# sevagh/demucs.cpp

Hardware: AMD Instinct MI355X
Metric: audio-sec/s (xRT) htdemucs-4s 44.1kHz stereo, ~4-min track with overlap-add (BASELINE configs[2]) (higher is better)
Workload: dtype f32 (exact bf16x3 operand split, fp32 accumulate)

## Files before the change

demucs_cpp_amd/csrc/api.cpp:

```cpp
#include "api_internal.h"

#include <algorithm>
#include <atomic>
#include <cstdarg>
#include <cstdio>
#include <cstdlib>
#include <cmath>
#include <cstring>
#include <cctype>
#include <cerrno>
#include <climits>
#include <fcntl.h>
#include <pthread.h>
#include <signal.h>
#include <sys/mman.h>
#include <sys/stat.h>
#include <unistd.h>

using namespace dmx;

static thread_local std::string g_err;
int dmx_fail(int code, const char *fmt, ...)
{
    char buf[1024];
// ... 108 lines not shown
    float *dx = nullptr;
    unsigned short *dp = nullptr;
    HIPCHK(hipMalloc((void **)&dx, sizeof(float) * (size_t)n));
    hipError_t e = hipMalloc((void **)&dp, sizeof(unsigned short) * 3 * (size_t)n);
    if (e == hipSuccess)
        e = hipMemcpy(dx, x, sizeof(float) * (size_t)n, hipMemcpyHostToDevice);
    if (e == hipSuccess)
    {
        launch_split3h_debug(dx, n, scale_exp, dp, nullptr);
        e = hipMemcpy(planes, dp, sizeof(unsigned short) * 3 * (size_t)n, hipMemcpyDeviceToHost);
    }
    (void)hipFree(dx);
    if (dp)
        (void)hipFree(dp);
    if (e != hipSuccess)
        return fail(DMX_ERR_HIP, "dmx_debug_split_activations_fp16: %s", hipGetErrorString(e));
    return DMX_OK;
}

static void fill_gemm_geometry(GemmArgs &k, const IGemm &g)
{
    k.xBS = g.xBatchStride;
    k.B = g.B, k.P1 = g.P1, k.P0 = g.P0, k.L1 = g.L1, k.L0 = g.L0, k.Cin = g.Cin;
    k.S1 = g.S1, k.stride1 = g.stride1, k.dil1 = g.dil1, k.pad1 = g.pad1;
    k.seg0 = g.seg0, k.stride0 = g.stride0, k.pad0 = g.pad0, k.K = g.K, k.Kp = g.Kp;
    k.pro = g.pro, k.G0 = g.G0;
    k.N = g.N, k.Np = g.Np;
    k.epi = g.epi, k.act = g.act, k.yBS = g.yBatchStride, k.ldy = g.ldy;
    k.NB = g.NB, k.tableScale = g.tableScale;
    k.Lout = g.Lout, k.Cout = g.Cout, k.trS = g.trS, k.trOff = g.trOff;
    k.kvCol0 = g.kvCol0, k.kvT = g.kvT, k.kvH = g.kvH, k.kvHs = g.kvHs;
    k.M = (i64)g.B * g.P1 * g.P0;
}

static bool split_ok_model(const dmx_ctx *c, const dmx_model *m, const IGemm &g);
static bool split_ok(const dmx_ctx *c, const IGemm &g) { return split_ok_model(c, c->m, g); }
static bool split_ok_model(const dmx_ctx *c, const dmx_model *m, const IGemm &g)
{
    if (c->gemm == DMX_GEMM_F32 || !m->dWb)
        return false;
    GemmArgs k{};
    fill_gemm_geometry(k, g);
    k.Wb1 = m->dWb + g.w_w, k.Wb2 = m->dWb + m->blobFloats + 512 + g.w_w;
    if (launch_igemm_split(g.cfg, k, nullptr, true) != 0)
        return false;
    const i64 lo = g.w_w, hi = g.w_w + (i64)g.Np * g.Kp;
    auto it = std::lower_bound(m->inexactW.begin(), m->inexactW.end(), lo);
    return it == m->inexactW.end() || *it >= hi;
}

static int split_kind_model(const dmx_ctx *c, const dmx_model *m, const IGemm &g)
{
    if (!split_ok_model(c, m, g))
        return 0;
    if (c->gemm != DMX_GEMM_FP16X3 || !m->dWh || !g.hterms)
        return 1;
    GemmArgs k{};
    fill_gemm_geometry(k, g);
    k.Wb1 = k.Wb2 = m->dWh;
    if (launch_igemm_split(g.cfg, k, nullptr, true, 1) != 0)
        return 1;
    const i64 lo = g.w_w, hi = g.w_w + (i64)g.Np * g.Kp;
    auto it = std::lower_bound(m->inexactH.begin(), m->inexactH.end(), lo);
    return (it == m->inexactH.end() || *it >= hi) ? 2 : 1;
}
static int split_kind(const dmx_ctx *c, const IGemm &g) { return split_kind_model(c, c->m, g); }

static int upload_failed(dmx_model *m, hipError_t e)
{
    for (void *p : {(void *)m->dW, (void *)m->dWb, (void *)m->dWh})
        if (p)
            (void)hipFree(p);
    m->dW = nullptr, m->dWb = nullptr, m->dWh = nullptr;
    return fail(DMX_ERR_HIP, "dmx_model_load: weight upload failed: %s", hipGetErrorString(e));
}

int dmx_model_upload(dmx_model *m, const float *blob)
{
    HIPCHK(hipSetDevice(m->device));
    HIPCHK(hipMalloc((void **)&m->dW, m->blobFloats * sizeof(float) + 1024));
    hipError_t e = hipMemset(reinterpret_cast<char *>(m->dW) + m->blobFloats * sizeof(float), 0, 1024);
    if (e == hipSuccess)
        e = hipMemcpy(m->dW, blob, m->blobFloats * sizeof(float), hipMemcpyHostToDevice);
    if (e != hipSuccess)
        return upload_failed(m, e);
    {
        std::vector<unsigned short> planes(2 * m->blobFloats + 1024, 0);
        m->inexactW.clear();
        for (size_t i = 0; i < m->blobFloats; ++i)
            if (!dmx_split_weight(blob[i], planes[i], planes[m->blobFloats + 512 + i]))
                m->inexactW.push_back((i64)i);
// ... 1602 lines not shown
extern "C" int dmx_debug_n_ops(const dmx_ctx *c)
{
    if (!c)
        return 0;
    auto it = c->plans.find(c->maxBatch);
    return it == c->plans.end() ? 0 : (int)it->second->ops.size();
}

static void op_work(const Op &op, const char *&kernel, double &flops, double &bytes)
{
    static const char *cfgNames[] = {"igemm_128x128", "igemm_64x64", "igemm_128x96", "igemm_128x48", "igemm_256x16", "igemm_128x32",
                                     "igemm_128x64",  "igemm_64x128", "dgemm_direct", "igemm_64x64", "igemm_64x96", "igemm_64x48",
                                     "igemm_64x32",   "igemm_64x64",  "igemm_128x16", "igemm_32x128", "igemm_32x64", "igemm_256x128", "igemm_256x128w4", "igemm_lin256x128", "igemm_256x96"};
    static_assert(sizeof(cfgNames) / sizeof(cfgNames[0]) == kNumTileCfgs, "one label per tile configuration");
    flops = bytes = 0;
    kernel = "?";
    switch (op.kind)
    {
    case OP_IGEMM:
    {
        const IGemm &g = op.g;
        const double M = (double)g.B * g.P1 * g.P0;
        kernel = cfgNames[g.cfg];
        if (g.split)
        {
            static const char *splitNames[kNumTileCfgs] = {"igemm_split_128x128", nullptr, "igemm_split_128x96", "igemm_split_128x48", nullptr, "igemm_split_128x32d", "igemm_split_128x64d",
                                                            "igemm_split_64x128", nullptr, "igemm_split_64x64", "igemm_split_64x96", "igemm_split_64x48",
                                                            "igemm_split_128x32d", "igemm_split_128x64d", nullptr, "igemm_split_32x128", "igemm_split_32x64", nullptr, nullptr,
                                                            nullptr, nullptr};
            if (splitNames[g.cfg])
                kernel = splitNames[g.cfg];
            if (g.split == 2)
                kernel = g.cfg == 0 ? "igemm_splith_128x128" : g.cfg == 7 ? "igemm_splith_64x128" : kernel;
            else if (g.cfg == 0 || g.cfg == 2)
            {
                GemmArgs k{};
                fill_gemm_geometry(k, g);
                k.rowstat = g.rowstat >= 0 ? reinterpret_cast<float *>(1) : nullptr;
                const int wide = igemm_split_is_wide(g.cfg, k);
                if (wide)
                    kernel = wide == 256 ? "igemm_split_128x256" : wide == 192 ? "igemm_split_128x192" : "igemm_split_128x96d";
            }
        }
        flops = 2.0 * M * g.N * g.K;
        double in = (double)g.B * g.L1 * g.L0 * g.Cin, w = (double)g.N * g.K, out = 0;
        if (g.epi == EPI_LINEAR || g.epi == EPI_SCALE_RES)
            out = M * g.N;
        else if (g.epi == EPI_KPL || g.epi == EPI_VT)
            out = M * g.N;
        else if (g.epi == EPI_GLU || g.epi == EPI_GN_GLU_SCALE_RES)
            out = M * g.N / 2;
        else if (g.epi == EPI_TRCONV)
            out = (double)g.B * g.P1 * g.Lout * g.Cout;
        double res = g.res >= 0 ? out : 0;
        bytes = 4.0 * (in + w + out + res);
        break;
    }
    case OP_ATTENTION:
    {
        const Attention &t = op.at;
        kernel = t.split ? "attention_split" : "attention";
        flops = 4.0 * t.B * t.H * (double)t.Tq * t.Tk * t.hs;
        bytes = 4.0 * t.B * t.H * t.hs * (2.0 * t.Tq + 2.0 * t.Tk);
        break;
    }
    case OP_DCONV_ROW:
    {
        const DconvRow &r = op.dr;
        const double M = (double)r.B * r.T * r.F, hp = (r.hid + 3) / 4 * 4;
        kernel = "dconv_row";
        flops = 2.0 * (2.0 * M * hp * 3.0 * r.C + 2.0 * M * (hp + 2) * hp + 2.0 * M * 2.0 * r.C * hp);
        bytes = 4.0 * 2.0 * M * r.C;
        break;
    }
// ... 120 lines not shown
```

demucs_cpp_amd/csrc/igemm_common.h:

```cpp
#pragma once
#include "kernels.h"

namespace dmx
{

typedef float f32x4 __attribute__((ext_vector_type(4)));
typedef float f32x2 __attribute__((ext_vector_type(2)));
typedef unsigned u32x4 __attribute__((ext_vector_type(4)));
typedef unsigned u32x2 __attribute__((ext_vector_type(2)));
typedef __bf16 bf16x2 __attribute__((ext_vector_type(2)));
typedef __bf16 bf16x8 __attribute__((ext_vector_type(8)));

__device__ __forceinline__ float gelu_f(float v) { return dmx_gelu(v); }
__device__ __forceinline__ float sigmoid_f(float v) { return __builtin_amdgcn_rcpf(1.0f + __expf(-v)); }
__device__ __forceinline__ float f4c(const f32x4 &v, int c) { return v[c]; }
__device__ __forceinline__ float4 ld4z(const float *ptr, bool ok, const float *zero)
{
    const f32x4 v = *reinterpret_cast<const f32x4 *>(ok ? ptr : zero);
    return make_float4(v[0], v[1], v[2], v[3]);
}

__device__ __forceinline__ void load_to_lds_b128(const float *gptr, float4 *lds_base)
{
#if defined(__HIP_DEVICE_COMPILE__)
// ... 272 lines not shown
                addrs_B();
            return;
        }
        if (c < 2)
            addrs_A_general(c);
        if (c == 2)
            addrs_B();
    }
    __device__ __forceinline__ f32x4 transform(f32x4 v, int i, bool ok, const f32x4 &gW, const f32x4 &gB) const
    {
        if (PRO != PRO_NONE)
        {
            if (PRO == PRO_AFFINE)
            {
                v.x = (v.x - aMean[i]) * aScale[i];
                v.y = (v.y - aMean[i]) * aScale[i];
                v.z = (v.z - aMean[i]) * aScale[i];
                v.w = (v.w - aMean[i]) * aScale[i];
            }
            if (PRO == PRO_GN_GELU)
            {
                v.x = gelu_f((v.x - aMean[i]) * aScale[i] * gW.x + gB.x);
                v.y = gelu_f((v.y - aMean[i]) * aScale[i] * gW.y + gB.y);
                v.z = gelu_f((v.z - aMean[i]) * aScale[i] * gW.z + gB.z);
                v.w = gelu_f((v.w - aMean[i]) * aScale[i] * gW.w + gB.w);
            }
            if (!ok)
                v = f32x4{0.f, 0.f, 0.f, 0.f};
        }
        return v;
    }
};

template <int WAVES_N, int WMF, int WNF, int EPI, int NT, int SSEG = 1, typename RowInfo>
__device__ __forceinline__ void igemm_epilogue(const GemmArgs &p, f32x4 (&acc)[WMF][WNF], RowInfo rowinfo, float2 (*rsum)[WAVES_N * SSEG], i64 m0,
                                               int n0, unsigned tileN, int wm, int wn, int BM)
{
    static_assert(WNF % SSEG == 0, "whole fragments per statistics run");
    const int tid = threadIdx.x, lane = tid & 63;
    const int l15 = lane & 15, kq = lane >> 4;
    if constexpr (EPI == EPI_VT)
    {
        const int nt = p.kvT >> 6;
        constexpr int IS = (WMF % 2 == 0) ? 2 : 1;
#pragma unroll
        for (int i = 0; i < WMF; i += IS)
        {
            const i64 m = m0 + wm * (WMF * 16) + i * 16 + 4 * kq;
            if (m >= p.M)
                continue;
            const unsigned b = (unsigned)m / (unsigned)p.kvT, t = (unsigned)m - b * (unsigned)p.kvT;
            const unsigned tt = t & 63u, slot = 4u * (tt >> 5) + ((tt >> 2) & 3u), half = (tt >> 4) & 1u;
#pragma unroll
            for (int j = 0; j < WNF; ++j)
            {
                const int n = n0 + wn * (WNF * 16) + j * 16 + l15;
                if (n >= p.N)
                    continue;
                const float bv = p.bias[n];
                const unsigned head = (unsigned)n / (unsigned)p.kvHs, dim = (unsigned)n - head * (unsigned)p.kvHs;
                unsigned short *dst = p.kvPl + ((((i64)b * p.kvH + head) * nt + (t >> 6)) * p.kvHs + dim) * 64 + slot * 8;
                unsigned h1[2 * IS], h2[2 * IS], h3[2 * IS];
#pragma unroll
                for (int u = 0; u < IS; ++u)
                {
                    split3_pk(acc[i + u][j][0] + bv, acc[i + u][j][1] + bv, h1[2 * u], h2[2 * u], h3[2 * u]);
                    split3_pk(acc[i + u][j][2] + bv, acc[i + u][j][3] + bv, h1[2 * u + 1], h2[2 * u + 1], h3[2 * u + 1]);
                }
                if constexpr (IS == 2)
// ... 41 lines not shown
                            *reinterpret_cast<float4 *>(p.Y + m * p.ldy + nb + 16 * u + 4 * kq) = v[u];
                    continue;
                }
                unsigned h[3][2][2];
#pragma unroll
                for (int u = 0; u < 2; ++u)
                {
                    split3_pk(v[u].x, v[u].y, h[0][u][0], h[1][u][0], h[2][u][0]);
                    split3_pk(v[u].z, v[u].w, h[0][u][1], h[1][u][1], h[2][u][1]);
                }
                const int nn = nb + 16 * (kq & 1) + 8 * (kq >> 1);
                unsigned short *dst = p.kvPl + m * (i64)(p.kvH * p.kvHs) + (nn - p.kvCol0);
#pragma unroll
                for (int pl = 0; pl < 3; ++pl)
                {
                    const u32x2 s0 = __builtin_amdgcn_permlane16_swap(h[pl][0][0], h[pl][1][0], false, false);
                    const u32x2 s1 = __builtin_amdgcn_permlane16_swap(h[pl][0][1], h[pl][1][1], false, false);
                    if (rowOk && nn < p.N)
                        *reinterpret_cast<u32x4 *>(dst + pl * p.kvPlane) = u32x4{s0[0], s1[0], s0[1], s1[1]};
                }
            }
        }
        return;
    }
    const bool wantStats = p.rowstat != nullptr;
    const int colBase = n0 + wn * (WNF * 16) + 4 * kq;
    float4 biasv[WNF], scalev[WNF], gnWv[WNF], gnBv[WNF];
    int trR[WNF], trC[WNF];
#pragma unroll
    for (int j = 0; j < WNF; ++j)
    {
        const int n = colBase + j * 16;
        const float4 z = make_float4(0.f, 0.f, 0.f, 0.f);
        biasv[j] = ld4z(p.bias + n, n < p.N, p.zero);
        scalev[j] = gnWv[j] = gnBv[j] = z;
        trR[j] = trC[j] = 0;
        if (EPI == EPI_TRCONV)
        {
            trR[j] = n / p.Cout;
            trC[j] = n - trR[j] * p.Cout;
        }
        if (EPI == EPI_SCALE_RES && n < p.N)
            scalev[j] = *reinterpret_cast<const float4 *>(p.scale + n);
        if (EPI == EPI_GN_GLU_SCALE_RES && n < p.N)
        {
            gnWv[j] = *reinterpret_cast<const float4 *>(p.epiW + n);
            gnBv[j] = *reinterpret_cast<const float4 *>(p.epiB + n);
            if ((j & 1) == 0)
                scalev[j] = *reinterpret_cast<const float4 *>(p.scale + (n >> 5) * 16 + (n & 15));
        }
    }

    constexpr int G = (16 / WNF) < 1 ? 1 : ((16 / WNF) > WMF ? WMF : (16 / WNF));
    int4 riA[G];
    float4 resA[G][WNF];
    float meanA[G], scA[G];
    i64 offsA[G][WNF];
#pragma unroll
    for (int g0 = 0; g0 < WMF; g0 += G)
    {
#pragma unroll
    for (int ig = 0; ig < G; ++ig)
    {
        const int i = g0 + ig;
        if (i >= WMF)
            break;
        const int rl = wm * (WMF * 16) + i * 16 + l15;
// ... 6 lines not shown
        for (int j = 0; j < WNF; ++j)
            resA[ig][j] = make_float4(0.f, 0.f, 0.f, 0.f);
        if (EPI == EPI_LINEAR || EPI == EPI_SCALE_RES)
        {
            if ((EPI == EPI_LINEAR && p.res) || EPI == EPI_SCALE_RES)
            {
#pragma unroll
                for (int j = 0; j < WNF; ++j)
                {
                    const int n = colBase + j * 16;
                    if (rowOk && n < p.N)
                        resA[ig][j] = *reinterpret_cast<const float4 *>(p.res + m * p.ldy + n);
                }
            }
        }
        else if (EPI == EPI_GLU || EPI == EPI_GN_GLU_SCALE_RES)
        {
            if (EPI == EPI_GN_GLU_SCALE_RES && rowOk)
            {
                meanA[ig] = p.epiStats[ri.w * 4];
                scA[ig] = p.epiStats[ri.w * 4 + 1];
            }
#pragma unroll
            for (int j = 0; j < WNF; j += 2)
            {
                const int na = colBase + j * 16;
                const int c = (na >> 5) * 16 + (na & 15);
                if (rowOk && na + 16 < p.N)
                {
                    if (EPI == EPI_GN_GLU_SCALE_RES)
                        resA[ig][j] = *reinterpret_cast<const float4 *>(p.res + m * p.ldy + c);
                    else if (p.table)
                    {
                        const float4 tv = *reinterpret_cast<const float4 *>(p.table + (i64)ri.z * (p.N >> 1) + c);
                        resA[ig][j] = make_float4(p.tableScale * tv.x, p.tableScale * tv.y, p.tableScale * tv.z, p.tableScale * tv.w);
                    }
                }
            }
        }
        else if (EPI == EPI_TRCONV)
        {
#pragma unroll
            for (int j = 0; j < WNF; ++j)
            {
                const int n = colBase + j * 16;
                const int jj = p.trS * ri.z + trR[j] - p.trOff;
                const i64 off = (rowOk && n < p.N && jj >= 0 && jj < p.Lout) ? (i64)ri.x * p.yBS + ((i64)ri.y * p.Lout + jj) * p.ldy + trC[j] : -1;
                offsA[ig][j] = off;
                if (p.res && off >= 0)
                    resA[ig][j] = *reinterpret_cast<const float4 *>(p.res + off);
            }
        }
    }
    __builtin_amdgcn_s_waitcnt(0x0F70);

#pragma unroll
    for (int ig = 0; ig < G; ++ig)
    {
        const int i = g0 + ig;
        if (i >= WMF)
            break;
        const int rl = wm * (WMF * 16) + i * 16 + l15;
        const int4 ri = riA[ig];
        const bool rowOk = ri.w >= 0;
        const i64 m = m0 + rl;
        float s = 0.f, ss = 0.f;
        float sSeg[SSEG], ssSeg[SSEG];
// ... 161 lines not shown
```

demucs_cpp_amd/csrc/igemm_split.hip:

```cpp
#include "igemm_common.h"
#include <cstdio>
#include <cstdlib>
#include <type_traits>

namespace dmx
{

__device__ __forceinline__ int swz(int row) { return (0x1320 >> (((row >> 2) & 3) * 4)) & 3; }

template <int WAVES_M, int WAVES_N, int WMF, int WNF, int PRO, int EPI, bool LIN>
__global__ __launch_bounds__(256, 2) void igemm_split_kernel(const GemmArgs p)
{
    constexpr int KT = 32;
    constexpr int BM = WAVES_M * WMF * 16;
    constexpr int BN = WAVES_N * WNF * 16;
    constexpr int LPR = 8;
    constexpr int RP = 256 / LPR;
    constexpr int AR = BM / RP;
    constexpr int BR = (BN + RP - 1) / RP;
    constexpr int BRP = BR * RP;
    static_assert(WAVES_M * WAVES_N == 4, "256 threads");
    static_assert(BM % RP == 0, "BM multiple of the staging pass");

    __shared__ u32x4 Ap0[3][BM][4], Ap1[3][BM][4];
// ... 386 lines not shown
            iteration(set1);
    }
    __syncthreads();
    if constexpr (ARITH == 1)
    {
#pragma unroll
        for (int i = 0; i < WMF; ++i)
        {
            if constexpr (EPI == EPI_VT)
            {
                float inv[4];
#pragma unroll
                for (int r = 0; r < 4; ++r)
                    inv[r] = p.rowScale[2 * min(m0 + wave * (WMF * 16) + i * 16 + 4 * kq + r, p.M - 1) + 1];
#pragma unroll
                for (int j = 0; j < WNF; ++j)
#pragma unroll
                    for (int r = 0; r < 4; ++r)
                        acc[i][j][r] *= inv[r];
            }
            else
            {
#pragma unroll
                for (int j = 0; j < WNF; ++j)
#pragma unroll
                    for (int r = 0; r < 4; ++r)
                        acc[i][j][r] *= aInv[i];
            }
        }
    }
    igemm_epilogue<1, WMF, WNF, EPI, 256, 2>(p, acc, rowinfo_of, rsum, m0, n0, tileN, wave, 0, BM);
}

template <int WNF, int EPI, bool GEN>
__global__ __launch_bounds__(256, WNF == 2 ? 4 : WNF <= 6 ? 3 : 2) void igemm_split_linw_kernel(const GemmArgs p)
{
    constexpr int KT = 32, WMF = 2, BM = 128, BN = 16 * WNF, NG = WNF / 2;
    constexpr int PW = WNF / 2;
    static_assert(WNF == 16 || WNF == 12 || WNF == 6 || WNF == 4 || WNF == 2,
                  "128 x 256 / 128 x 192 / 128 x 96 (N = 96 layers: three workgroups per CU) / 128 x 64 (the last transposed conv of the "
                  "frequency branch, N = 64: three) / 128 x 32 (the C = 192 DConv K1, N = 24: four)");
    __shared__ u32x4 Bp[2][2][BN][4];

    const int tid = threadIdx.x, lane = tid & 63, wave = tid >> 6;
    const int l15 = lane & 15, kq = lane >> 4;
    unsigned tileM, tileN;
    if (!tile_of_block(p, tileM, tileN))
        return;
    const i64 m0 = (i64)tileM * BM;
    const int n0 = (int)tileN * BN;
    auto rowinfo_of = [&](int r) -> int4 { return row_info(p, m0 + r); };

    unsigned aOff[WMF];
    const float *aRow[WMF];
    unsigned aMask[WMF];
    int gS1 = 0, gOffb = kq * 8, gTapC = 0, gTapOff = kq * 8;
    const int rowLenI = p.L0 * p.Cin;
    {
        const i64 rowLen = (i64)p.L0 * p.Cin;
#pragma unroll
        for (int i = 0; i < WMF; ++i)
        {
            const i64 m = min(m0 + wave * (WMF * 16) + i * 16 + l15, p.M - 1);
            const int4 ri = row_info(p, m);
            aOff[i] = 0, aRow[i] = p.X, aMask[i] = 0;
            if constexpr (GEN)
            {
                const int taps0 = p.seg0 / p.Cin;
                const int in1_0 = ri.y * p.stride1 - p.pad1;
                const int e0 = (ri.z * p.stride0 - p.pad0) * p.Cin;
                aRow[i] = p.X + (i64)ri.x * p.xBS + (i64)in1_0 * rowLen + e0;
                unsigned m0bits = 0;
                for (int t0 = 0; t0 < taps0; ++t0)
                {
                    const int e = e0 + t0 * p.Cin;
                    m0bits |= (e >= 0 && e < rowLenI ? 1u : 0u) << t0;
                }
                for (int s = 0; s < p.S1; ++s)
                {
                    const int in1 = in1_0 + s * p.dil1;
                    if (in1 >= 0 && in1 < p.L1)
                        aMask[i] |= m0bits << (s * taps0);
                }
            }
            else
                aOff[i] = (unsigned)(((i64)ri.x * p.xBS + (i64)ri.y * rowLen + (i64)ri.z * p.stride0 * p.Cin) * 4 + kq * 32);
        }
        if constexpr (GEN)
        {
            if (p.S1 > 1)
                while (gOffb >= p.seg0)
                {
                    gOffb -= p.seg0;
                    ++gS1;
                }
            while (gTapOff >= p.Cin)
            {
                gTapOff -= p.Cin;
// ... 56 lines not shown
            aRaw[SET][i][0] = *reinterpret_cast<const f32x4 *>(src);
            aRaw[SET][i][1] = *reinterpret_cast<const f32x4 *>(src + 16);
            aOff[i] += KT * 4;
        }
    };
    auto split_block = [&](auto setTag, int i) {
        constexpr int SET = decltype(setTag)::value;
        const f32x4 lo = aRaw[SET][i][0], hi = aRaw[SET][i][1];
        unsigned h1[4], h2[4], h3[4];
        split3_pk(lo[0], lo[1], h1[0], h2[0], h3[0]);
        split3_pk(lo[2], lo[3], h1[1], h2[1], h3[1]);
        split3_pk(hi[0], hi[1], h1[2], h2[2], h3[2]);
        split3_pk(hi[2], hi[3], h1[3], h2[3], h3[3]);
        u32x4 q1{h1[0], h1[1], h1[2], h1[3]}, q2{h2[0], h2[1], h2[2], h2[3]}, q3{h3[0], h3[1], h3[2], h3[3]};
        asm volatile("" : "+v"(q1), "+v"(q2), "+v"(q3));
        aPl[SET][i][0] = q1;
        aPl[SET][i][1] = q2;
        aPl[SET][i][2] = q3;
    };

    f32x4 acc[WMF][WNF];
#pragma unroll
    for (int i = 0; i < WMF; ++i)
#pragma unroll
        for (int j = 0; j < WNF; ++j)
            acc[i][j] = f32x4{0.f, 0.f, 0.f, 0.f};

    const std::integral_constant<int, 0> set0{};
    const std::integral_constant<int, 1> set1{};
    const int nk = (p.Kp + 31) >> 5;
    load_A(set0);
    load_A(set1);
    dma_B(0);
    split_block(set0, 0);
    split_block(set0, 1);
    asm volatile("s_waitcnt vmcnt(0)" ::: "memory");
    __syncthreads();
    const int fslot = kq ^ swz(l15);
    auto iteration = [&](auto parTag) {
        constexpr int PAR = decltype(parTag)::value;
        const std::integral_constant<int, PAR ^ 1> other{};
        load_A(parTag);
        __builtin_amdgcn_sched_barrier(0);
        dma_B(PAR ^ 1);
        u32x4 b1[2][2], b2[2][2];
        auto read_group = [&](int g) {
#pragma unroll
            for (int u = 0; u < 2; ++u)
            {
                const int r = (2 * g + u) * 16 + l15;
                b1[g & 1][u] = Bp[PAR][0][r][fslot];
                b2[g & 1][u] = Bp[PAR][1][r][fslot];
            }
        };
        auto term = [&](int g, u32x4(&b)[2], int plane) {
#pragma unroll
            for (int i = 0; i < WMF; ++i)
#pragma unroll
                for (int u = 0; u < 2; ++u)
                {
                    if constexpr (EPI == EPI_VT)
                        acc[i][2 * g + u] = __builtin_amdgcn_mfma_f32_16x16x32_bf16(__builtin_bit_cast(bf16x8, aPl[PAR][i][plane]), __builtin_bit_cast(bf16x8, b[u]), acc[i][2 * g + u], 0, 0, 0);
                    else
                        acc[i][2 * g + u] = __builtin_amdgcn_mfma_f32_16x16x32_bf16(__builtin_bit_cast(bf16x8, b[u]), __builtin_bit_cast(bf16x8, aPl[PAR][i][plane]), acc[i][2 * g + u], 0, 0, 0);
                }
        };
        read_group(0);
#pragma unroll
        for (int g = 0; g < NG; ++g)
        {
            if (g + 1 < NG)
                read_group(g + 1);
            term(g, b1[g & 1], 2);
            term(g, b2[g & 1], 1);
            if (g == (WNF == 16 ? 2 : WNF == 12 ? 1 : 0))
                split_block(other, 0);
            if (g == (WNF == 16 ? 5 : WNF == 12 ? 4 : WNF == 6 ? 2 : WNF == 4 ? 1 : 0))
                split_block(other, 1);
            term(g, b2[g & 1], 0);
            term(g, b1[g & 1], 1);
            term(g, b1[g & 1], 0);
            __builtin_amdgcn_sched_barrier(0);
        }
        asm volatile("s_waitcnt vmcnt(0)" ::: "memory");
        __syncthreads();
    };
    for (int kt = 0; kt < nk; kt += 2)
    {
        iteration(set0);
        if (kt + 1 < nk)
            iteration(set1);
    }

    if constexpr (EPI == EPI_KPL || EPI == EPI_VT)
    {
        float2(*none)[1] = nullptr;
        igemm_epilogue<1, WMF, WNF, EPI, 256>(p, acc, rowinfo_of, none, m0, n0, tileN, wave, 0, BM);
    }
    else if constexpr (WNF == 2)
    {
        float2(*rsum)[1] = reinterpret_cast<float2(*)[1]>(&Bp[0][0][0][0]);
        igemm_epilogue<1, WMF, WNF, EPI, 256>(p, acc, rowinfo_of, rsum, m0, n0, tileN, wave, 0, BM);
    }
    else if constexpr (GEN || WNF != 16)
    {
        float2(*none)[1] = nullptr;
        constexpr int JC = WNF % 4 == 0 ? 4 : 6;
#pragma unroll
        for (int jc = 0; jc < WNF; jc += JC)
        {
            f32x4 part[WMF][JC];
#pragma unroll
            for (int i = 0; i < WMF; ++i)
#pragma unroll
                for (int j = 0; j < JC; ++j)
                    part[i][j] = acc[i][jc + j];
            igemm_epilogue<1, WMF, JC, EPI, 256>(p, part, rowinfo_of, none, m0, n0 + 16 * jc, tileN, wave, 0, BM);
        }
    }
    else
    {
        static_assert(EPI == EPI_LINEAR || EPI == EPI_SCALE_RES, "plain linear layers");
        const bool hasRes = EPI == EPI_SCALE_RES || p.res != nullptr;
        const bool wantStats = p.rowstat != nullptr;
        float2(*rsum)[4] = reinterpret_cast<float2(*)[4]>(&Bp[0][0][0][0]);
#pragma unroll
        for (int jc = 0; jc < WNF; jc += 4)
        {
            float4 biasv[4], scalev[4], resv[WMF][4];
#pragma unroll
            for (int j = 0; j < 4; ++j)
            {
                const int n = n0 + (jc + j) * 16 + 4 * kq;
                biasv[j] = *reinterpret_cast<const float4 *>(p.bias + n);
                if (EPI == EPI_SCALE_RES)
                    scalev[j] = *reinterpret_cast<const float4 *>(p.scale + n);
#pragma unroll
                for (int i = 0; i < WMF; ++i)
                {
                    const i64 m = m0 + wave * (WMF * 16) + i * 16 + l15;
                    resv[i][j] = make_float4(0.f, 0.f, 0.f, 0.f);
                    if (hasRes && m < p.M)
                        resv[i][j] = *reinterpret_cast<const float4 *>(p.res + m * p.ldy + n);
                }
            }
#pragma unroll
            for (int i = 0; i < WMF; ++i)
            {
                const int rl = wave * (WMF * 16) + i * 16 + l15;
                const i64 m = m0 + rl;
// ... 129 lines not shown
{
    const i64 pairs = (n + 1) / 2;
    hipLaunchKernelGGL(split3h_debug_kernel, dim3((unsigned)((pairs + 255) / 256)), dim3(256), 0, s, d_x, n, ldexpf(1.0f, sexp), d_planes);
}

static constexpr double kWideMinRounds = 2.5;
static bool wide_tile_pays(const GemmArgs &a, int mode)
{
    if (a.N % 256 != 0 || a.Np != a.N || a.Kp % 32 != 0 || mode == 2 || mode == 0 || (a.rowstat && a.NB != a.N / 128))
        return false;
    if (mode == 3)
        return true;
    const i64 tm = (a.M + 127) / 128;
    return (double)(((tm + 7) / 8) * (a.N / 256)) / 64.0 >= kWideMinRounds;
}

static int wide_conv_width(const GemmArgs &a, int pro, int epi, int mode)
{
    if (mode == 0 || mode == 2 || pro != PRO_NONE || !(epi == EPI_LINEAR || epi == EPI_GLU || epi == EPI_TRCONV) || a.rowstat)
        return 0;
    const int wnf = a.N % 256 == 0 ? 16 : a.N % 192 == 0 ? 12 : a.N == 96 ? 6 : 0;
    if (!wnf || a.Np != a.N || a.Kp % 16 != 0 || a.Cin % 8 != 0 || a.seg0 % a.Cin != 0 || a.seg0 < 32 || a.S1 * (a.seg0 / a.Cin) > 32 ||
        (i64)a.S1 * a.dil1 * a.L0 * a.Cin + a.seg0 >= (1ll << 31) || (epi == EPI_TRCONV && a.Cout % 4 != 0))
        return 0;
    if (mode == 3)
        return wnf;
    if (mode == 4 && wnf == 6)
        return 0;
    if (wnf == 6)
        return wnf;
    const i64 tm = (a.M + 127) / 128;
    return (double)(((tm + 7) / 8) * (a.N / (16 * wnf))) / 64.0 >= (a.N == 192 ? 0.6 : 0.9) ? wnf : 0;
}
template <int EPI>
static void launch_wide_conv(GemmArgs a, int wnf, hipStream_t s)
{
    a.tilesM = (unsigned)((a.M + 127) / 128);
    a.tilesN = (unsigned)(a.N / (16 * wnf));
    const dim3 grid(8u * ((a.tilesM + 7u) / 8u) * a.tilesN);
    if (wnf == 16)
        hipLaunchKernelGGL((igemm_split_linw_kernel<16, EPI, true>), grid, dim3(256), 0, s, a);
    else if (wnf == 12)
        hipLaunchKernelGGL((igemm_split_linw_kernel<12, EPI, true>), grid, dim3(256), 0, s, a);
    else
        hipLaunchKernelGGL((igemm_split_linw_kernel<6, EPI, true>), grid, dim3(256), 0, s, a);
}

static int launch_split_narrow(int cfg, const GemmArgs &a0, hipStream_t s, int arith, bool dry)
{
    const GemmArgs &a = a0;
    const int np = (cfg == 5 || cfg == 12) ? 32 : 64;
    if (arith != 0 || a.pro != PRO_NONE || !(a.epi == EPI_LINEAR || (a.epi == EPI_TRCONV && np == 64)) || (a.epi == EPI_LINEAR && a.res) || a.N > np || a.Np != np ||
        a.Kp % 16 != 0 || a.Cin % 8 != 0 || a.Cin <= 0 || a.seg0 % a.Cin != 0 || a.seg0 < 32 || a.S1 * (a.seg0 / a.Cin) > 32 ||
        (i64)a.S1 * a.dil1 * a.L0 * a.Cin + a.seg0 >= (1ll << 31) || a.NB != 1 || (a.epi == EPI_TRCONV && (a.rowstat || a.Cout % 4 != 0)) ||
        (np == 64 && a.rowstat))
        return -1;
    if (dry)
        return 0;
    GemmArgs k = a;
    k.tilesM = (unsigned)((k.M + 127) / 128);
    k.tilesN = 1;
    k.xcdMap = 1;
    k.dP0 = make_fastdiv((unsigned)k.P0), k.dP1 = make_fastdiv((unsigned)k.P1);
    const dim3 grid(8u * ((k.tilesM + 7u) / 8u));
    if (np == 32)
        hipLaunchKernelGGL((igemm_split_linw_kernel<2, EPI_LINEAR, true>), grid, dim3(256), 0, s, k);
    else if (a.epi == EPI_LINEAR)
        hipLaunchKernelGGL((igemm_split_linw_kernel<4, EPI_LINEAR, true>), grid, dim3(256), 0, s, k);
    else
        hipLaunchKernelGGL((igemm_split_linw_kernel<4, EPI_TRCONV, true>), grid, dim3(256), 0, s, k);
    return 0;
}

template <int WM_, int WN_, int MF, int NF, int PRO, int EPI>
static int launch_split_one(const GemmArgs &a0, hipStream_t s, int arith, bool dry)
{
    if (dry && arith == 0 && EPI != EPI_KPL && EPI != EPI_VT)
        return 0;
    constexpr int BM = WM_ * MF * 16, BN = WN_ * NF * 16;
    GemmArgs a = a0;
    a.tilesM = (unsigned)((a.M + BM - 1) / BM);
    a.tilesN = (unsigned)((a.N + BN - 1) / BN);
    a.xcdMap = 1;
    a.dP0 = make_fastdiv((unsigned)a.P0), a.dP1 = make_fastdiv((unsigned)a.P1);
    const unsigned blocks = 8u * ((a.tilesM + 7u) / 8u) * a.tilesN;
    const bool lin = gemm_is_linear(a, PRO, EPI, 32) && ((i64)a.B * a.xBS + 64) * 4 < (1ll << 32) &&
                     ((i64)(a.Wb2 - a.Wb1) + (i64)a.Np * a.Kp + 64) * 2 < (1ll << 32);
    if constexpr (EPI == EPI_KPL || EPI == EPI_VT)
    {
        if constexpr (PRO == PRO_NONE && WM_ == 2 && WN_ == 2 && NF == 4 && MF >= 2)
            if (lin)
            {
                if (dry)
                    return 0;
                static const int mode = [] { const char *e = getenv("DMX_SPLIT_LIN"); return e ? atoi(e) : 1; }();
                if (arith == 1)
                    hipLaunchKernelGGL((igemm_split_lin_kernel<MF / 2, 8, EPI, 1>), dim3(blocks), dim3(256), 0, s, a);
                else if (MF == 4 && wide_tile_pays(a, mode == 0 ? 1 : mode))
                {
                    a.tilesN = (unsigned)(a.N / 256);
                    hipLaunchKernelGGL((igemm_split_linw_kernel<16, EPI, false>), dim3(8u * ((a.tilesM + 7u) / 8u) * a.tilesN), dim3(256), 0, s, a);
// ... 45 lines not shown
                return -1;
            hipLaunchKernelGGL((igemm_split_kernel<WM_, WN_, MF, NF, PRO, EPI, true>), dim3(blocks), dim3(256), 0, s, a);
            return 0;
        }
    }
    if (arith == 1)
        return -1;
    if constexpr (PRO == PRO_NONE && EPI == EPI_TRCONV && ((WM_ == 2 && WN_ == 2 && MF == 4 && NF == 4) || (WM_ == 4 && WN_ == 1 && MF == 2 && NF == 6)))
    {
        static const int mode = [] { const char *e = getenv("DMX_SPLIT_LIN"); return e ? atoi(e) : 1; }();
        if (const int wnf = wide_conv_width(a, PRO, EPI, mode))
        {
            launch_wide_conv<EPI>(a, wnf, s);
            return 0;
        }
    }
    if constexpr (EPI != EPI_KPL && EPI != EPI_VT)
        hipLaunchKernelGGL((igemm_split_kernel<WM_, WN_, MF, NF, PRO, EPI, false>), dim3(blocks), dim3(256), 0, s, a);
    return 0;
}

int igemm_split_is_wide(int cfg, const GemmArgs &a)
{
    static const int mode = [] { const char *e = getenv("DMX_SPLIT_LIN"); return e ? atoi(e) : 1; }();
    if (cfg != 0 && cfg != 2)
        return 0;
    const bool lin = gemm_is_linear(a, a.pro, a.epi, 32) && ((i64)a.B * a.xBS + 64) * 4 < (1ll << 32);
    if (cfg == 0 && lin && (a.epi == EPI_LINEAR || a.epi == EPI_SCALE_RES || a.epi == EPI_KPL || a.epi == EPI_VT) &&
        wide_tile_pays(a, (a.epi == EPI_KPL || a.epi == EPI_VT) && mode == 0 ? 1 : mode))
        return 256;
    if (lin && a.epi == EPI_LINEAR && a.N % 256 == 0)
        return 0;
    return 16 * wide_conv_width(a, a.pro, a.epi, mode);
}

int launch_igemm_split(int cfg, const GemmArgs &a, hipStream_t s, bool dry, int arith)
{
    if (a.M >= (1ll << 31) - 256 || !a.Wb1 || !a.Wb2)
        return -1;
#define DMX_CASE(cfgid, WM_, WN_, MF, NF, PRO, EPI) \
    case (cfgid * 100 + PRO * 10 + EPI):           \
        return launch_split_one<WM_, WN_, MF, NF, PRO, EPI>(a, s, arith, dry);
    if (cfg == 5 || cfg == 12 || cfg == 6 || cfg == 13)
        return launch_split_narrow(cfg, a, s, arith, dry);
    switch (cfg * 100 + a.pro * 10 + a.epi)
    {
        DMX_CASE(0, 2, 2, 4, 4, PRO_NONE, EPI_LINEAR)
        DMX_CASE(0, 2, 2, 4, 4, PRO_NONE, EPI_SCALE_RES)
        DMX_CASE(0, 2, 2, 4, 4, PRO_NONE, EPI_GLU)
        DMX_CASE(0, 2, 2, 4, 4, PRO_NONE, EPI_TRCONV)
        DMX_CASE(7, 2, 2, 2, 4, PRO_NONE, EPI_LINEAR)
        DMX_CASE(7, 2, 2, 2, 4, PRO_NONE, EPI_SCALE_RES)
        DMX_CASE(7, 2, 2, 2, 4, PRO_NONE, EPI_GLU)
        DMX_CASE(7, 2, 2, 2, 4, PRO_NONE, EPI_TRCONV)
        DMX_CASE(0, 2, 2, 4, 4, PRO_NONE, EPI_KPL)
        DMX_CASE(0, 2, 2, 4, 4, PRO_NONE, EPI_VT)
        DMX_CASE(7, 2, 2, 2, 4, PRO_NONE, EPI_KPL)
        DMX_CASE(7, 2, 2, 2, 4, PRO_NONE, EPI_VT)
        DMX_CASE(2, 4, 1, 2, 6, PRO_NONE, EPI_LINEAR)
        DMX_CASE(2, 4, 1, 2, 6, PRO_NONE, EPI_GLU)
        DMX_CASE(2, 4, 1, 2, 6, PRO_NONE, EPI_TRCONV)
        DMX_CASE(15, 2, 2, 1, 4, PRO_NONE, EPI_LINEAR)
        DMX_CASE(15, 2, 2, 1, 4, PRO_NONE, EPI_SCALE_RES)
        DMX_CASE(15, 2, 2, 1, 4, PRO_NONE, EPI_GLU)
        DMX_CASE(15, 2, 2, 1, 4, PRO_NONE, EPI_TRCONV)
        DMX_CASE(9, 2, 2, 2, 2, PRO_NONE, EPI_LINEAR)
// ... 20 lines not shown
```

demucs_cpp_amd/csrc/kernels.h:

```cpp
#pragma once
#include "plan.h"
#include <hip/hip_runtime.h>
#include <cstdlib>

namespace dmx
{

struct FastDiv
{
    unsigned magic, shift;
};
inline FastDiv make_fastdiv(unsigned d)
{
    FastDiv f;
    f.magic = 0;
    f.shift = 0;
    if (d == 0)
        d = 1;
    if ((d & (d - 1)) == 0)
    {
        while ((1u << f.shift) < d)
            ++f.shift;
        return f;
    }
// ... 27 lines not shown
    const float *table;
    float tableScale;
    int Lout, Cout;
    int trS, trOff;
    const float *rowScale;
    unsigned short *kvPl;
    i64 kvPlane;
    int kvCol0, kvT, kvH, kvHs;
    i64 M;
    const float *zero;
    unsigned tilesM, tilesN;
    FastDiv dP0, dP1;
    int xcdMap;
};

int launch_dgemm(const GemmArgs &a, hipStream_t s, bool dry = false);

struct DconvRowArgs
{
    float *x;
    int B, T, F, C, hid;
    const float *img[2];
    float eps;
    const float *zero;
    int rowsPerXcd;
    double n1, invN1, invN1m1, n2, invN2, invN2m1;
};
int launch_dconv_row(const DconvRowArgs &a, hipStream_t s, bool dry = false);

int launch_igemm(int cfg, const GemmArgs &a, hipStream_t s, bool dry = false);
int launch_igemm_lin256(const GemmArgs &a, hipStream_t s, bool dry = false);
int launch_igemm_split(int cfg, const GemmArgs &a, hipStream_t s, bool dry = false, int arith = 0);
int igemm_split_is_wide(int cfg, const GemmArgs &a);
void launch_rowscale(const GemmArgs &a, float *out, hipStream_t s);
void launch_split3h_debug(const float *d_x, i64 n, int sexp, unsigned short *d_planes, hipStream_t s);
void launch_split3_debug(const float *d_x, i64 n, unsigned short *d_planes, hipStream_t s);

struct ReduceArgs
{
    const float *rowstat;
    float *out;
    int B, R, NB, G0;
    double count;
    int mode;
    float eps;
    double *scratch;
    int nchunk;
};
void launch_stats_reduce(const ReduceArgs &a, hipStream_t s);

struct StftArgs
{
    const float *mix;
    float *x, *rowstat, *rowstatT;
    int B, T, seg, pad;
    const float *window, *twiddle;
};
void launch_stft(const StftArgs &a, hipStream_t s);

struct LnArgs
{
    const float *x;
    float *y;
    int rows, D, rowsPerBatch;
    const float *w, *b, *pe;
    float eps;
// ... 205 lines not shown
```

Before: 3173.

## Add resident-weight short-K variants of the split wide conv GEMM

Adds a short-K path to the split bf16x3 linw kernel for GLU and transposed-conv epilogues when K spans only 2, 3 or 5 tiles. All weight k-tiles are loaded into LDS once up front, which removes the per-iteration B DMA, the vmcnt waits and the barriers, and the K loop is fully unrolled. Bias and, for one GLU form, the positional table are prefetched into registers before the main loop. The larger LDS footprint lowers the occupancy bound, and a small-grid heuristic and an env switch gate the new path.

```diff
diff --git a/demucs_cpp_amd/csrc/api.cpp b/demucs_cpp_amd/csrc/api.cpp
--- a/demucs_cpp_amd/csrc/api.cpp
+++ b/demucs_cpp_amd/csrc/api.cpp
@@ -164,6 +164,11 @@
     k.kvCol0 = g.kvCol0, k.kvT = g.kvT, k.kvH = g.kvH, k.kvHs = g.kvHs;
     k.M = (i64)g.B * g.P1 * g.P0;
 }
+static void fill_gemm_presence(GemmArgs &k, const IGemm &g)
+{
+    k.res = g.res >= 0 ? reinterpret_cast<float *>(1) : nullptr;
+    k.rowstat = g.rowstat >= 0 ? reinterpret_cast<float *>(1) : nullptr;
+}
 
 static bool split_ok_model(const dmx_ctx *c, const dmx_model *m, const IGemm &g);
 static bool split_ok(const dmx_ctx *c, const IGemm &g) { return split_ok_model(c, c->m, g); }
@@ -173,6 +178,7 @@
         return false;
     GemmArgs k{};
     fill_gemm_geometry(k, g);
+    fill_gemm_presence(k, g);
     k.Wb1 = m->dWb + g.w_w, k.Wb2 = m->dWb + m->blobFloats + 512 + g.w_w;
     if (launch_igemm_split(g.cfg, k, nullptr, true) != 0)
         return false;
@@ -189,6 +195,7 @@
         return 1;
     GemmArgs k{};
     fill_gemm_geometry(k, g);
+    fill_gemm_presence(k, g);
     k.Wb1 = k.Wb2 = m->dWh;
     if (launch_igemm_split(g.cfg, k, nullptr, true, 1) != 0)
         return 1;
@@ -1857,14 +1864,16 @@
                 kernel = splitNames[g.cfg];
             if (g.split == 2)
                 kernel = g.cfg == 0 ? "igemm_splith_128x128" : g.cfg == 7 ? "igemm_splith_64x128" : kernel;
-            else if (g.cfg == 0 || g.cfg == 2)
+            else if (g.cfg == 0 || g.cfg == 2 || g.cfg == 6 || g.cfg == 13)
             {
                 GemmArgs k{};
                 fill_gemm_geometry(k, g);
-                k.rowstat = g.rowstat >= 0 ? reinterpret_cast<float *>(1) : nullptr;
+                fill_gemm_presence(k, g);
                 const int wide = igemm_split_is_wide(g.cfg, k);
                 if (wide)
                     kernel = wide == 256 ? "igemm_split_128x256" : wide == 192 ? "igemm_split_128x192" : "igemm_split_128x96d";
+                if (igemm_split_is_shortk(g.cfg, k))
+                    kernel = "igemm_split_shortk";
             }
         }
         flops = 2.0 * M * g.N * g.K;
diff --git a/demucs_cpp_amd/csrc/igemm_common.h b/demucs_cpp_amd/csrc/igemm_common.h
--- a/demucs_cpp_amd/csrc/igemm_common.h
+++ b/demucs_cpp_amd/csrc/igemm_common.h
@@ -328,9 +328,20 @@
     }
 };
 
-template <int WAVES_N, int WMF, int WNF, int EPI, int NT, int SSEG = 1, typename RowInfo>
+struct EpiNoPre
+{
+    static constexpr bool kHave = false, kTab = false;
+};
+template <int WMF, int WNF, bool TABLE>
+struct EpiPre
+{
+    static constexpr bool kHave = true, kTab = TABLE;
+    float4 bias[WNF];
+    float4 tab[TABLE ? WMF : 1][(WNF + 1) / 2];
+};
+template <int WAVES_N, int WMF, int WNF, int EPI, int NT, int SSEG = 1, typename RowInfo, typename Pre = EpiNoPre>
 __device__ __forceinline__ void igemm_epilogue(const GemmArgs &p, f32x4 (&acc)[WMF][WNF], RowInfo rowinfo, float2 (*rsum)[WAVES_N * SSEG], i64 m0,
-                                               int n0, unsigned tileN, int wm, int wn, int BM)
+                                               int n0, unsigned tileN, int wm, int wn, int BM, const Pre &pre = Pre{})
 {
     static_assert(WNF % SSEG == 0, "whole fragments per statistics run");
     const int tid = threadIdx.x, lane = tid & 63;
@@ -438,7 +449,10 @@
     {
         const int n = colBase + j * 16;
         const float4 z = make_float4(0.f, 0.f, 0.f, 0.f);
-        biasv[j] = ld4z(p.bias + n, n < p.N, p.zero);
+        if constexpr (Pre::kHave)
+            biasv[j] = pre.bias[j];
+        else
+            biasv[j] = ld4z(p.bias + n, n < p.N, p.zero);
         scalev[j] = gnWv[j] = gnBv[j] = z;
         trR[j] = trC[j] = 0;
         if (EPI == EPI_TRCONV)
@@ -511,7 +525,11 @@
                         resA[ig][j] = *reinterpret_cast<const float4 *>(p.res + m * p.ldy + c);
                     else if (p.table)
                     {
-                        const float4 tv = *reinterpret_cast<const float4 *>(p.table + (i64)ri.z * (p.N >> 1) + c);
+                        float4 tv;
+                        if constexpr (Pre::kTab)
+                            tv = pre.tab[i][j >> 1];
+                        else
+                            tv = *reinterpret_cast<const float4 *>(p.table + (i64)ri.z * (p.N >> 1) + c);
                         resA[ig][j] = make_float4(p.tableScale * tv.x, p.tableScale * tv.y, p.tableScale * tv.z, p.tableScale * tv.w);
                     }
                 }
diff --git a/demucs_cpp_amd/csrc/igemm_split.hip b/demucs_cpp_amd/csrc/igemm_split.hip
--- a/demucs_cpp_amd/csrc/igemm_split.hip
+++ b/demucs_cpp_amd/csrc/igemm_split.hip
@@ -442,15 +442,23 @@
     igemm_epilogue<1, WMF, WNF, EPI, 256, 2>(p, acc, rowinfo_of, rsum, m0, n0, tileN, wave, 0, BM);
 }
 
-template <int WNF, int EPI, bool GEN>
-__global__ __launch_bounds__(256, WNF == 2 ? 4 : WNF <= 6 ? 3 : 2) void igemm_split_linw_kernel(const GemmArgs p)
+constexpr int linw_min_workgroups(int WNF, int NKT)
+{
+    const int byRegs = WNF == 2 ? 4 : WNF <= 6 ? 3 : 2;
+    const int byLds = NKT ? (160 * 1024) / (NKT * 2 * 16 * WNF * 64) : 4;
+    return byLds < byRegs ? (byLds < 1 ? 1 : byLds) : byRegs;
+}
+template <int WNF, int EPI, bool GEN, int NKT = 0, bool TAB = false>
+__global__ __launch_bounds__(256, linw_min_workgroups(WNF, NKT)) void igemm_split_linw_kernel(const GemmArgs p)
 {
     constexpr int KT = 32, WMF = 2, BM = 128, BN = 16 * WNF, NG = WNF / 2;
+    static_assert(NKT == 0 || (GEN && (EPI == EPI_GLU || EPI == EPI_TRCONV) && WNF != 2 && WNF != 16), "resident weights: the short-K conv forms");
+    static_assert(!TAB || (NKT > 0 && EPI == EPI_GLU), "table prefetch: the GLU rewrites of the resident-weight form");
     constexpr int PW = WNF / 2;
     static_assert(WNF == 16 || WNF == 12 || WNF == 6 || WNF == 4 || WNF == 2,
                   "128 x 256 / 128 x 192 / 128 x 96 (N = 96 layers: three workgroups per CU) / 128 x 64 (the last transposed conv of the "
                   "frequency branch, N = 64: three) / 128 x 32 (the C = 192 DConv K1, N = 24: four)");
-    __shared__ u32x4 Bp[2][2][BN][4];
+    __shared__ u32x4 Bp[NKT ? NKT : 2][2][BN][4];
 
     const int tid = threadIdx.x, lane = tid & 63, wave = tid >> 6;
     const int l15 = lane & 15, kq = lane >> 4;
@@ -464,6 +472,7 @@
     unsigned aOff[WMF];
     const float *aRow[WMF];
     unsigned aMask[WMF];
+    EpiPre<WMF, WNF, TAB> pre;
     int gS1 = 0, gOffb = kq * 8, gTapC = 0, gTapOff = kq * 8;
     const int rowLenI = p.L0 * p.Cin;
     {
@@ -474,6 +483,16 @@
             const i64 m = min(m0 + wave * (WMF * 16) + i * 16 + l15, p.M - 1);
             const int4 ri = row_info(p, m);
             aOff[i] = 0, aRow[i] = p.X, aMask[i] = 0;
+            if constexpr (TAB)
+            {
+#pragma unroll
+                for (int j = 0; j < WNF; j += 2)
+                {
+                    const int na = n0 + j * 16 + 4 * kq;
+                    const f32x4 tv = *reinterpret_cast<const f32x4 *>(p.table + (i64)ri.z * (p.N >> 1) + ((na >> 5) * 16 + (na & 15)));
+                    pre.tab[i][j >> 1] = make_float4(tv[0], tv[1], tv[2], tv[3]);
+                }
+            }
             if constexpr (GEN)
             {
                 const int taps0 = p.seg0 / p.Cin;
@@ -596,25 +615,40 @@
     load_A(set0);
     load_A(set1);
     dma_B(0);
+    if constexpr (NKT > 0)
+    {
+#pragma unroll
+        for (int kt = 1; kt < NKT; ++kt)
+            dma_B(kt);
+#pragma unroll
+        for (int j = 0; j < WNF; ++j)
+        {
+            const int n = n0 + j * 16 + 4 * kq;
+            pre.bias[j] = ld4z(p.bias + n, n < p.N, p.zero);
+        }
+    }
     split_block(set0, 0);
     split_block(set0, 1);
     asm volatile("s_waitcnt vmcnt(0)" ::: "memory");
     __syncthreads();
     const int fslot = kq ^ swz(l15);
-    auto iteration = [&](auto parTag) {
+    auto iteration = [&](auto parTag, int kt) {
         constexpr int PAR = decltype(parTag)::value;
         const std::integral_constant<int, PAR ^ 1> other{};
-        load_A(parTag);
+        const int img = NKT ? kt : PAR;
+        if (!NKT || kt + 2 < NKT)
+            load_A(parTag);
         __builtin_amdgcn_sched_barrier(0);
-        dma_B(PAR ^ 1);
+        if constexpr (NKT == 0)
+            dma_B(PAR ^ 1);
         u32x4 b1[2][2], b2[2][2];
         auto read_group = [&](int g) {
 #pragma unroll
             for (int u = 0; u < 2; ++u)
             {
                 const int r = (2 * g + u) * 16 + l15;
-                b1[g & 1][u] = Bp[PAR][0][r][fslot];
-                b2[g & 1][u] = Bp[PAR][1][r][fslot];
+                b1[g & 1][u] = Bp[img][0][r][fslot];
+                b2[g & 1][u] = Bp[img][1][r][fslot];
             }
         };
         auto term = [&](int g, u32x4(&b)[2], int plane) {
@@ -637,24 +671,38 @@
                 read_group(g + 1);
             term(g, b1[g & 1], 2);
             term(g, b2[g & 1], 1);
-            if (g == (WNF == 16 ? 2 : WNF == 12 ? 1 : 0))
+            if (g == (WNF == 16 ? 2 : WNF == 12 ? 1 : 0) && (!NKT || kt + 1 < NKT))
                 split_block(other, 0);
-            if (g == (WNF == 16 ? 5 : WNF == 12 ? 4 : WNF == 6 ? 2 : WNF == 4 ? 1 : 0))
+            if (g == (WNF == 16 ? 5 : WNF == 12 ? 4 : WNF == 6 ? 2 : WNF == 4 ? 1 : 0) && (!NKT || kt + 1 < NKT))
                 split_block(other, 1);
             term(g, b2[g & 1], 0);
             term(g, b1[g & 1], 1);
             term(g, b1[g & 1], 0);
             __builtin_amdgcn_sched_barrier(0);
         }
-        asm volatile("s_waitcnt vmcnt(0)" ::: "memory");
-        __syncthreads();
-    };
-    for (int kt = 0; kt < nk; kt += 2)
-    {
-        iteration(set0);
-        if (kt + 1 < nk)
-            iteration(set1);
-    }
+        if constexpr (NKT == 0)
+        {
+            asm volatile("s_waitcnt vmcnt(0)" ::: "memory");
+            __syncthreads();
+        }
+    };
+    if constexpr (NKT > 0)
+    {
+#pragma unroll
+        for (int kt = 0; kt < NKT; kt += 2)
+        {
+            iteration(set0, kt);
+            if (kt + 1 < NKT)
+                iteration(set1, kt + 1);
+        }
+    }
+    else
+        for (int kt = 0; kt < nk; kt += 2)
+        {
+            iteration(set0, kt);
+            if (kt + 1 < nk)
+                iteration(set1, kt + 1);
+        }
 
     if constexpr (EPI == EPI_KPL || EPI == EPI_VT)
     {
@@ -679,7 +727,24 @@
 #pragma unroll
                 for (int j = 0; j < JC; ++j)
                     part[i][j] = acc[i][jc + j];
-            igemm_epilogue<1, WMF, JC, EPI, 256>(p, part, rowinfo_of, none, m0, n0 + 16 * jc, tileN, wave, 0, BM);
+            if constexpr (NKT > 0)
+            {
+                EpiPre<WMF, JC, TAB> pp;
+#pragma unroll
+                for (int j = 0; j < JC; ++j)
+                    pp.bias[j] = pre.bias[jc + j];
+                if constexpr (TAB)
+                {
+#pragma unroll
+                    for (int i = 0; i < WMF; ++i)
+#pragma unroll
+                        for (int j = 0; j < JC; j += 2)
+                            pp.tab[i][j >> 1] = pre.tab[i][(jc + j) >> 1];
+                }
+                igemm_epilogue<1, WMF, JC, EPI, 256>(p, part, rowinfo_of, none, m0, n0 + 16 * jc, tileN, wave, 0, BM, pp);
+            }
+            else
+                igemm_epilogue<1, WMF, JC, EPI, 256>(p, part, rowinfo_of, none, m0, n0 + 16 * jc, tileN, wave, 0, BM);
         }
     }
     else
@@ -875,12 +940,45 @@
     const i64 tm = (a.M + 127) / 128;
     return (double)(((tm + 7) / 8) * (a.N / (16 * wnf))) / 64.0 >= (a.N == 192 ? 0.6 : 0.9) ? wnf : 0;
 }
+static constexpr double kShortK5MinRounds = 10.0;
+static int shortk_tiles(const GemmArgs &a, int wnf, int epi)
+{
+    static const int on = [] { const char *e = getenv("DMX_SPLIT_SHORTK"); return e ? atoi(e) : 1; }();
+    if (!on || a.res || a.rowstat || a.Np != a.N || a.Kp % 16 != 0)
+        return 0;
+    const int nk = (a.Kp + 31) / 32;
+    if (nk == 5 && (double)((((a.M + 127) / 128) + 7) / 8) / 64.0 < kShortK5MinRounds)
+        return 0;
+    if (epi == EPI_GLU && ((wnf == 6 && (nk == 2 || nk == 5)) || (wnf == 12 && nk == 3)))
+        return nk;
+    if (epi == EPI_TRCONV && (wnf == 4 || wnf == 6) && nk == 3)
+        return nk;
+    return 0;
+}
 template <int EPI>
 static void launch_wide_conv(GemmArgs a, int wnf, hipStream_t s)
 {
     a.tilesM = (unsigned)((a.M + 127) / 128);
     a.tilesN = (unsigned)(a.N / (16 * wnf));
     const dim3 grid(8u * ((a.tilesM + 7u) / 8u) * a.tilesN);
+    if constexpr (EPI == EPI_GLU || EPI == EPI_TRCONV)
+        if (const int nkt = shortk_tiles(a, wnf, EPI))
+        {
+            if constexpr (EPI == EPI_GLU)
+            {
+                if (wnf == 12)
+                    hipLaunchKernelGGL((igemm_split_linw_kernel<12, EPI_GLU, true, 3>), grid, dim3(256), 0, s, a);
+                else if (nkt == 5)
+                    hipLaunchKernelGGL((igemm_split_linw_kernel<6, EPI_GLU, true, 5>), grid, dim3(256), 0, s, a);
+                else if (a.table)
+                    hipLaunchKernelGGL((igemm_split_linw_kernel<6, EPI_GLU, true, 2, true>), grid, dim3(256), 0, s, a);
+                else
+                    hipLaunchKernelGGL((igemm_split_linw_kernel<6, EPI_GLU, true, 2>), grid, dim3(256), 0, s, a);
+            }
+            else
+                hipLaunchKernelGGL((igemm_split_linw_kernel<6, EPI_TRCONV, true, 3>), grid, dim3(256), 0, s, a);
+            return;
+        }
     if (wnf == 16)
         hipLaunchKernelGGL((igemm_split_linw_kernel<16, EPI, true>), grid, dim3(256), 0, s, a);
     else if (wnf == 12)
@@ -910,6 +1008,8 @@
         hipLaunchKernelGGL((igemm_split_linw_kernel<2, EPI_LINEAR, true>), grid, dim3(256), 0, s, k);
     else if (a.epi == EPI_LINEAR)
         hipLaunchKernelGGL((igemm_split_linw_kernel<4, EPI_LINEAR, true>), grid, dim3(256), 0, s, k);
+    else if (shortk_tiles(k, 4, EPI_TRCONV))
+        hipLaunchKernelGGL((igemm_split_linw_kernel<4, EPI_TRCONV, true, 3>), grid, dim3(256), 0, s, k);
     else
         hipLaunchKernelGGL((igemm_split_linw_kernel<4, EPI_TRCONV, true>), grid, dim3(256), 0, s, k);
     return 0;
@@ -1021,6 +1121,16 @@
     if (lin && a.epi == EPI_LINEAR && a.N % 256 == 0)
         return 0;
     return 16 * wide_conv_width(a, a.pro, a.epi, mode);
+}
+
+int igemm_split_is_shortk(int cfg, const GemmArgs &a)
+{
+    if (cfg == 6 || cfg == 13)
+        return launch_split_narrow(cfg, a, nullptr, 0, true) == 0 && a.epi == EPI_TRCONV ? shortk_tiles(a, 4, EPI_TRCONV) : 0;
+    const int wide = igemm_split_is_wide(cfg, a);
+    if (wide != 96 && wide != 192 && wide != 256)
+        return 0;
+    return (a.epi == EPI_GLU || a.epi == EPI_TRCONV) ? shortk_tiles(a, wide / 16, a.epi) : 0;
 }
 
 int launch_igemm_split(int cfg, const GemmArgs &a, hipStream_t s, bool dry, int arith)
diff --git a/demucs_cpp_amd/csrc/kernels.h b/demucs_cpp_amd/csrc/kernels.h
--- a/demucs_cpp_amd/csrc/kernels.h
+++ b/demucs_cpp_amd/csrc/kernels.h
@@ -83,6 +83,7 @@
 int launch_igemm_lin256(const GemmArgs &a, hipStream_t s, bool dry = false);
 int launch_igemm_split(int cfg, const GemmArgs &a, hipStream_t s, bool dry = false, int arith = 0);
 int igemm_split_is_wide(int cfg, const GemmArgs &a);
+int igemm_split_is_shortk(int cfg, const GemmArgs &a);
 void launch_rowscale(const GemmArgs &a, float *out, hipStream_t s);
 void launch_split3h_debug(const float *d_x, i64 n, int sexp, unsigned short *d_planes, hipStream_t s);
 void launch_split3_debug(const float *d_x, i64 n, unsigned short *d_planes, hipStream_t s);
```

Measured after the change: 3177 (median of 2 runs). Within noise of the previous version (+0.1%).
